# LeonhardFeiner/sparse_rcnn

Measured on AMD Instinct MI355X. Metric: active-voxels/sec fwd+bwd, ScanNet U-Net backbone, higher is better.
Workload: dtype f32

## Files before the change

### include/scn_mi355x.h

```cpp
#ifndef SCN_MI355X_H
#define SCN_MI355X_H

#include <stdint.h>

#ifdef __cplusplus
extern "C" {
#endif

#define SCN_OK 0
#define SCN_EINVAL 1
#define SCN_ESIZE 2
#define SCN_EHASH 3
#define SCN_EHIP 4

#define SCN_ABI_VERSION 5

#define SCN_F_RELU_IN 1
#define SCN_F_W_TRANSPOSED 2
#define SCN_F_OFF_REVERSE 4
#define SCN_F_RESIDUAL_LAST 8
#define SCN_F_SPLIT_SUM 16
#define SCN_F_TILE_ORDER_X 64
#define SCN_F_GEMM_V1 32

// ... 136 lines not shown
                         int flags, scn_stream_t stream);
int scn_wgrad_bias_rules_bf16(const uint16_t* X, int cin, const uint16_t* dY, int cout, const int32_t* in_rows,
                              const int32_t* out_rows, const int64_t* prefix_host, int n_off, float* dW, float* db,
                              uint32_t db_offsets, void* scratch, int flags, scn_stream_t stream);
int scn_wgrad_bias_rules(const float* X, int cin, const float* dY, int cout, const int32_t* in_rows,
                         const int32_t* out_rows, const int64_t* prefix_host, int n_off, float* dW, float* db,
                         uint32_t db_offsets, void* scratch, int flags, scn_stream_t stream);

int scn_wgrad_defer_begin(void);
int scn_wgrad_defer_flush(scn_stream_t stream);
int scn_wgrad_step_begin(void);
int scn_wgrad_step_hold(int on);
int scn_wgrad_step_flush(scn_stream_t stream);
int scn_wgrad_step_discard(void);
void scn_wgrad_group_counts(int64_t out[4], int reset);
int64_t scn_wgrad_scratch_bytes2(int cin, int cout, const int64_t* prefix_host, int n_off);
int scn_wgrad_bias_rules2(const float* X0, const float* dY0, const float* X1, const float* dY1, int cin, int cout,
                          const int32_t* in_rows, const int32_t* out_rows, const int64_t* prefix_host, int n_off,
                          float* dW, float* db, uint32_t db_offsets, void* scratch, int flags, scn_stream_t stream);

int64_t scn_wgrad_scratch_bytes_n(int cin, int cout, const int64_t* prefix_host, int n_off, int n_prob);
int scn_wgrad_bias_rules_n(const float* const* Xs, const float* const* dYs, int n_prob, int cin, int cout,
                          const int32_t* in_rows, const int32_t* out_rows, const int64_t* prefix_host, int n_off,
                          float* dW, float* db, uint32_t db_offsets, void* scratch, int flags, scn_stream_t stream);
int scn_wgrad_bias_rules_n_bf16(const uint16_t* const* Xs, const uint16_t* const* dYs, int n_prob, int cin, int cout,
                               const int32_t* in_rows, const int32_t* out_rows, const int64_t* prefix_host, int n_off,
                               float* dW, float* db, uint32_t db_offsets, void* scratch, int flags, scn_stream_t stream);
int scn_wgrad_bias_rules2_bf16(const uint16_t* X0, const uint16_t* dY0, const uint16_t* X1, const uint16_t* dY1, int cin,
                               int cout, const int32_t* in_rows, const int32_t* out_rows, const int64_t* prefix_host,
                               int n_off, float* dW, float* db, uint32_t db_offsets, void* scratch, int flags,
// ... 311 lines not shown
```

### sparse_rcnn_amd/_lib.py

```python
from __future__ import annotations

import ctypes as C
import os

import torch

_HERE = os.path.dirname(os.path.abspath(__file__))
LIB_PATH = os.environ.get("SCN_MI355X_LIB") or os.path.join(_HERE, "libscn_mi355x.so")

_lib = None

p = C.c_void_p
i32, i64, f32 = C.c_int, C.c_int64, C.c_float

_SIGS = {
    "scn_abi_version": (C.c_int, []),
    "scn_last_error_string": (C.c_char_p, []),
    "scn_debug_set": (C.c_int, [C.c_char_p, C.c_char_p]),
    "scn_debug_get": (C.c_int, [C.c_char_p, C.POINTER(C.c_int), C.POINTER(i64)]),
    "scn_hash_capacity": (i64, [i64]),
    "scn_coords_to_i32": (C.c_int, [p, i64, p, p, C.POINTER(i64), p]),
    "scn_dedup_scratch_bytes": (i64, [i64]),
    "scn_dedup_build": (C.c_int, [p, i64, i32, p, p, i64, p, p, p, p, p, C.POINTER(i64), p]),
    "scn_dedup_launch": (C.c_int, [p, i64, i32, p, p, i64, p, p, p, p, p, p, p]),
# ... 42 lines not shown
    "scn_wgrad_rules": (C.c_int, [p, i32, p, i32, p, p, C.POINTER(i64), i32, p, p, i32, p]),
    "scn_gemm_table_bf16": (C.c_int, [p, i64, i32, p, i32, i64, p, p, p, p, p, i32, i32, p]),
    "scn_gemm_rules_bf16": (C.c_int, [p, i32, p, p, C.POINTER(i64), i32, p, p, p, p, i32, i32, p]),
    "scn_gemm_rows2": (C.c_int, [p, i32, p, i32, i64, p, p, p, p, p, i32, p, i32, i32, i32, p]),
    "scn_wgrad_rules_bf16": (C.c_int, [p, i32, p, i32, p, p, C.POINTER(i64), i32, p, p, i32, p]),
    "scn_wgrad_bias_rules": (C.c_int, [p, i32, p, i32, p, p, C.POINTER(i64), i32, p, p, C.c_uint32, p, i32, p]),
    "scn_wgrad_bias_rules_bf16": (C.c_int, [p, i32, p, i32, p, p, C.POINTER(i64), i32, p, p, C.c_uint32, p, i32, p]),
    "scn_wgrad_scratch_bytes2": (i64, [i32, i32, C.POINTER(i64), i32]),
    "scn_wgrad_defer_begin": (C.c_int, []),
    "scn_wgrad_defer_flush": (C.c_int, [p]),
    "scn_wgrad_step_begin": (C.c_int, []),
    "scn_wgrad_step_hold": (C.c_int, [i32]),
    "scn_wgrad_step_flush": (C.c_int, [p]),
    "scn_wgrad_step_discard": (C.c_int, []),
    "scn_wgrad_group_counts": (None, [C.POINTER(i64), i32]),
    "scn_wgrad_bias_rules2": (C.c_int, [p, p, p, p, i32, i32, p, p, C.POINTER(i64), i32, p, p, C.c_uint32, p, i32, p]),
    "scn_wgrad_bias_rules2_bf16": (C.c_int, [p, p, p, p, i32, i32, p, p, C.POINTER(i64), i32, p, p, C.c_uint32, p, i32, p]),
    "scn_wgrad_scratch_bytes_n": (i64, [i32, i32, C.POINTER(i64), i32, i32]),
    "scn_wgrad_bias_rules_n": (C.c_int, [C.POINTER(p), C.POINTER(p), i32, i32, i32, p, p, C.POINTER(i64), i32, p, p, C.c_uint32, p, i32, p]),
    "scn_wgrad_bias_rules_n_bf16": (C.c_int, [C.POINTER(p), C.POINTER(p), i32, i32, i32, p, p, C.POINTER(i64), i32, p, p, C.c_uint32, p, i32, p]),
    "scn_colsum": (C.c_int, [p, i64, i32, p, p, p]),
    "scn_colsum_bf16": (C.c_int, [p, i64, i32, p, p, p]),
    "scn_relu_fwd": (C.c_int, [p, i64, p, p]),
    "scn_relu_bwd": (C.c_int, [p, p, i64, p, p]),
    "scn_add": (C.c_int, [p, p, i64, p, p]),
    "scn_bn_scratch_bytes": (i64, [i32]),
    "scn_bn_stats": (C.c_int, [p, i64, i32, p, p, p, p]),
    "scn_bn_sums": (C.c_int, [p, i64, i32, p, p, p]),
    "scn_bn_bwd_reduce": (C.c_int, [p, p, i64, i32, p, p, f32, p, p, f32, p, p, p, p, p]),
    "scn_bn_bwd_apply": (C.c_int, [p, p, i64, i32, p, p, f32, p, p, f32, p, i64, p, p]),
# ... 212 lines not shown
```

### sparse_rcnn_amd/csrc/scn_common.h

```cpp
#pragma once
#include <hip/hip_runtime.h>
#include <atomic>
#include <stdint.h>
#include <stdio.h>
#include <string.h>

#include "../../include/scn_mi355x.h"

namespace scn {

extern thread_local char g_err[512];

inline int fail(int code, const char* fmt, const char* a = "", long long b = 0, long long c = 0) {
    snprintf(g_err, sizeof(g_err), fmt, a, b, c);
    return code;
}

#define SCN_HIP(expr)                                                                               \
    do {                                                                                            \
        hipError_t e_ = (expr);                                                                     \
        if (e_ != hipSuccess) {                                                                     \
            snprintf(scn::g_err, sizeof(scn::g_err), "%s failed: %s (%s:%d)", #expr,                \
                     hipGetErrorString(e_), __FILE__, __LINE__);                                    \
            return SCN_EHIP;                                                                        \
// ... 10 lines not shown
        }                                                                                           \
    } while (0)

#define SCN_REQUIRE(cond)                                                                           \
    do {                                                                                            \
        if (!(cond)) {                                                                              \
            snprintf(scn::g_err, sizeof(scn::g_err), "%s: requirement failed: %s", __func__, #cond); \
            return SCN_EINVAL;                                                                      \
        }                                                                                           \
    } while (0)

enum Switch {
    SW_TS_SPLIT, SW_TS_SPLIT_MAX, SW_TS_NO_TAIL, SW_TS_W_HALF, SW_TS_W_BOTH, SW_TB_NB, SW_TB_KH, SW_TB_STREAM,
    SW_TB_NO_XORDER, SW_TS_STREAM, SW_TSS_NW, SW_EXEC_DEFER_SUMS, SW_PYRAMID_V1, SW_PYRAMID_ONE_STREAM, SW_WD_NO_T3,
    SW_WGRAD_BF16_MFMA, SW_WGRAD_SPLITS, SW_WD_NO_EVEC, SW_PYRAMID_NO_BRICKS, SW_CU_BUDGET, SW_EXP_A, SW_EXP_B, SW_TS_NO_CHAIN, SW_TS_PROG, SW_TB_NO_BINS,
    SW_EXEC_GROUP_WGRAD, SW_EXEC_GROUP_STEP, SW_COUNT
};
struct SwitchVal { bool set = false; long long i = 0; double f = 0.0; };
SwitchVal sw(Switch s);
inline int cu_budget() { const SwitchVal v = sw(SW_CU_BUDGET); return (v.set && v.i >= 32 && v.i <= 256) ? (int)v.i : 256; }

struct DeviceOnce {
    std::atomic<uint64_t> mask{0};
    static int cur() { int d = 0; return (hipGetDevice(&d) == hipSuccess && d >= 0 && d < 64) ? d : -1; }
    bool needed() const { const int d = cur(); return d < 0 || !(mask.load(std::memory_order_acquire) & (1ull << d)); }
    void done() { const int d = cur(); if (d >= 0) mask.fetch_or(1ull << d, std::memory_order_release); }
};

int wgrad_defer_group(bool on);

inline hipStream_t S(scn_stream_t s) { return reinterpret_cast<hipStream_t>(s); }
// ... 44 lines not shown
```

### sparse_rcnn_amd/csrc/scn_debug.hip

```cpp
#include <stdlib.h>

#include <mutex>

#include "scn_common.h"

namespace scn {
namespace {
struct Entry { const char* name; SwitchVal v; };
Entry g_sw[SW_COUNT] = {
    {"SCN_TS_SPLIT", {}},        {"SCN_TS_SPLIT_MAX", {}},  {"SCN_TS_NO_TAIL", {}},       {"SCN_TS_W_HALF", {}},
    {"SCN_TS_W_BOTH", {}},       {"SCN_TB_NB", {}},         {"SCN_TB_KH", {}},            {"SCN_TB_STREAM", {}},
    {"SCN_TB_NO_XORDER", {}},    {"SCN_TS_STREAM", {}},     {"SCN_TSS_NW", {}},           {"SCN_EXEC_DEFER_SUMS", {}},
    {"SCN_PYRAMID_V1", {}},      {"SCN_PYRAMID_ONE_STREAM", {}}, {"SCN_WD_NO_T3", {}},    {"SCN_WGRAD_BF16_MFMA", {}},
    {"SCN_WGRAD_SPLITS", {}},    {"SCN_WD_NO_EVEC", {}},    {"SCN_PYRAMID_NO_BRICKS", {}},            {"SCN_CU_BUDGET", {}},
    {"SCN_EXP_A", {}},           {"SCN_EXP_B", {}},         {"SCN_TS_NO_CHAIN", {}},
    {"SCN_TS_PROG", {}},         {"SCN_TB_NO_BINS", {}},    {"SCN_EXEC_GROUP_WGRAD", {}},
    {"SCN_EXEC_GROUP_STEP", {}},
};
std::once_flag g_once;
std::mutex g_mu;

void assign(SwitchVal& v, const char* s) {
    v.set = s != nullptr;
    v.i = s ? atoll(s) : 0;
    v.f = s ? atof(s) : 0.0;
}
void load_env() {
    for (int k = 0; k < SW_COUNT; ++k) assign(g_sw[k].v, getenv(g_sw[k].name));
}
}

SwitchVal sw(Switch s) {
// ... 30 lines not shown
```

### sparse_rcnn_amd/csrc/scn_wgrad.hip

```cpp
#include <stdlib.h>

#include <string.h>
#include <mutex>
#include <vector>

#include "scn_common.h"

#ifndef WD_DEEP_ALL
#define WD_DEEP_ALL 1
#endif

using scn::S;
using scn::cdiv;

typedef float f32x4 __attribute__((ext_vector_type(4)));
#define MFMA16(a, b, c) __builtin_amdgcn_mfma_f32_16x16x4f32((a), (b), (c), 0, 0, 0)

#ifndef WD_EXP
#define WD_EXP 0
#endif
#ifndef WD_TIMELINE
#define WD_TIMELINE 0
#endif
#if WD_TIMELINE
// ... 43 lines not shown
            f[2 * j] = __uint_as_float(r[j] << 16);
            f[2 * j + 1] = __uint_as_float(r[j] & 0xffff0000u);
        }
    } else {
        f = r;
    }
    return f;
}

__device__ __forceinline__ void wd_range(const DPlan& plan, int ov, int o, int prob, long long& p_lo, long long& p_hi) {
    const long long p_shift = prob * plan.p_rules;
    p_lo = plan.rule_start[ov] - p_shift;
    p_hi = plan.rule_start[ov + 1] - p_shift;
}

template <int TA, int TB, bool QUAD, bool EDGE, bool IDENT, bool HB = false>
__global__ __launch_bounds__(256) void k_wgrad_direct(const float* __restrict__ X_0, int cin, const float* __restrict__ dY_0,
                                                      int cout, const int* __restrict__ in_rows,
                                                      const int* __restrict__ out_rows, DPlan plan,
                                                      float* __restrict__ slabs, int relu_in,
                                                      float* __restrict__ db_slabs, unsigned db_mask, int cout_pad,
                                                      WdOps more) {
    const int unit = blockIdx.x, zb = blockIdx.z;
#include "scn_wgrad_unit.inc"
}

#define WG_MAX_JOBS 6
#define WG_MAXV 54
#define WG_MAXR 27
struct GJob {
    const void* X[2]; const void* dY[2];
    const int* in_rows; const int* out_rows;
    float* slabs; float* db_slabs;
    long long per;
    int cin, cout, relu_in, cout_pad, n_off, n_real, nbi, nbj, units, kind;
    unsigned db_mask;
    int unit_start[WG_MAXV + 1];
    long long prefix[WG_MAXR + 1];
};
struct GroupJobs { int n; int block_start[WG_MAX_JOBS + 1]; GJob job[WG_MAX_JOBS]; };

__device__ __forceinline__ int wd_offset_of(const GJob& j, int unit, int lane) {
    const bool lo = lane < j.n_off && unit >= j.unit_start[lane + 1];
    return __builtin_amdgcn_readfirstlane(__popcll(__ballot(lo)));
}
__device__ __forceinline__ void wd_range(const GJob& j, int ov, int o, int prob, long long& p_lo, long long& p_hi) {
    p_lo = j.prefix[o];
    p_hi = j.prefix[o + 1];
}

#define WD_KIND(TA_, TB_, Q_, E_, I_, H_) \
    ((TA_) | ((TB_) << 3) | ((Q_) ? 1 << 6 : 0) | ((E_) ? 1 << 7 : 0) | ((I_) ? 1 << 8 : 0) | ((H_) ? 1 << 9 : 0))

// ... 5 lines not shown
    return j;
}
#define WG_CONST(T_, p_) ((const __attribute__((address_space(4))) T_*)(p_))
__device__ __forceinline__ int wg_find(const GroupTable& t, int b) {
    int lo = 0, hi = t.n;
    while (hi - lo > 1) {
        const int mid = (lo + hi) >> 1;
        if (b >= WG_CONST(int, t.block_start)[mid]) lo = mid; else hi = mid;
    }
    return lo;
}
__device__ __forceinline__ const GJob& wg_job(const GroupJobs& g, int j) { return g.job[j]; }
__device__ __forceinline__ int wg_start(const GroupJobs& g, int j) { return g.block_start[j]; }
__device__ __forceinline__ const GJob& wg_job(const GroupTable& t, int j) { return *(const GJob*)(WG_CONST(GJob, t.job) + j); }
__device__ __forceinline__ int wg_start(const GroupTable& t, int j) { return WG_CONST(int, t.block_start)[j]; }

template <int VAR, typename SRC = GroupJobs>
__global__ __launch_bounds__(256) __attribute__((amdgpu_waves_per_eu(VAR, VAR))) void k_wgrad_group(SRC g) {
    const int j = wg_find(g, (int)blockIdx.x);
    const GJob& J = wg_job(g, j);
    const int local = (int)blockIdx.x - wg_start(g, j);
    const int zb = local / J.units, unit = local - zb * J.units;
    const float* __restrict__ X_0 = (const float*)J.X[0];
    const float* __restrict__ dY_0 = (const float*)J.dY[0];
    const int cin = J.cin, cout = J.cout, relu_in = J.relu_in, cout_pad = J.cout_pad;
    const int* __restrict__ in_rows = J.in_rows;
    const int* __restrict__ out_rows = J.out_rows;
    float* __restrict__ slabs = J.slabs;
    float* __restrict__ db_slabs = J.db_slabs;
    const unsigned db_mask = J.db_mask;
    const GJob& plan = J;
    const GJob& more = J;
#define WG_UNIT(TA_, TB_, Q_, I_) \
    constexpr int TA = TA_, TB = TB_;  \
    constexpr bool QUAD = Q_, EDGE = false, IDENT = I_, HB = false;
    if constexpr (VAR == 4) {
        switch (J.kind) {
        case WD_KIND(2, 2, false, false, false, false): {
            WG_UNIT(2, 2, false, false)
#include "scn_wgrad_unit.inc"
        } break;
        case WD_KIND(2, 2, false, false, true, false): {
            WG_UNIT(2, 2, false, true)
#include "scn_wgrad_unit.inc"
        } break;
        default: break;
        }
    } else {
        switch (J.kind) {
        case WD_KIND(2, 2, false, false, false, false): {
// ... 36 lines not shown
            WG_UNIT(4, 4, false, true)
#include "scn_wgrad_unit.inc"
        } break;
        case WD_KIND(4, 4, true, false, false, false): {
            WG_UNIT(4, 4, true, false)
#include "scn_wgrad_unit.inc"
        } break;
        case WD_KIND(4, 4, true, false, true, false): {
            WG_UNIT(4, 4, true, true)
#include "scn_wgrad_unit.inc"
        } break;
        default: break;
        }
    }
#undef WG_UNIT
}


typedef short s16x4 __attribute__((ext_vector_type(4)));
typedef short s16x8 __attribute__((ext_vector_type(8)));
typedef __bf16 bf16x8 __attribute__((ext_vector_type(8)));
#define MFMAB32(a, b, c) __builtin_amdgcn_mfma_f32_16x16x32_bf16((a), (b), (c), 0, 0, 0)

__device__ __forceinline__ int wtb_off(int row, int ch) { return 256 * row + 16 * (ch ^ (((row & 3) << 2) | ((row >> 2) & 3))); }

template <int TA, int TB, bool IDENT>
__global__ __launch_bounds__(256) void k_wgrad_tb(const unsigned short* __restrict__ X_0, int cin,
                                                  const unsigned short* __restrict__ dY_0, int cout,
                                                  const int* __restrict__ in_rows, const int* __restrict__ out_rows,
                                                  DPlan plan, float* __restrict__ slabs, int relu_in,
// ... 148 lines not shown
                slab[(16 * (wi * TA + a) + 4 * kq + j) * CBJ + 16 * (wj * TB + b) + i] = acc[a][b][j];
    if (do_db && kq == 0) {
#pragma unroll
        for (int b = 0; b < TB; ++b) {
            const int c = co0 + 16 * (wj * TB + b) + i;
            if (c < cout_pad) db_slabs[(long long)unit * cout_pad + c] = dbacc[b][0];
        }
    }
}

struct SumArgs {
    const float* slabs; float* dW; const float* db_slabs; float* db;
    int unit_start[129];
    int n_off, n_real, cbi, cbj, nbi, nbj, cin, cout, cout_pad, main_blocks, G;
    unsigned db_mask;
};

template <int V, typename A>
__device__ __forceinline__ void wgradd_sum_body(const A& a, int block) {
    typedef typename Frag<V>::type vec_t;
    const float* __restrict__ slabs = a.slabs;
    const int cin = a.cin, cout = a.cout, G = a.G;
    if (block >= a.main_blocks) {
        const int cidx = block - a.main_blocks;
        const int prob = cidx / cout, co = cidx - prob * cout;
        float s = 0.f;
        for (int o = 0; o < a.n_real; ++o) {
            if (!((a.db_mask >> o) & 1u)) continue;
            const int ov = prob * a.n_real + o;
            for (int u = a.unit_start[ov] + threadIdx.x; u < a.unit_start[ov + 1]; u += 256)
                s += a.db_slabs[(long long)u * a.cout_pad + co];
        }
#pragma unroll
        for (int d = 32; d >= 1; d >>= 1) s += __shfl_down(s, d);
        __shared__ float w[4];
        if ((threadIdx.x & 63) == 0) w[threadIdx.x >> 6] = s;
        __syncthreads();
        if (threadIdx.x == 0) a.db[cidx] = (w[0] + w[1]) + (w[2] + w[3]);
        return;
    }
    __shared__ __attribute__((aligned(16))) float part[256 * V];
    const int per_block = 256 / G;
    const int el = threadIdx.x % per_block, g = threadIdx.x / per_block;
    const long long total = (long long)a.n_off * cin * (cout / V);
    const int cbi = a.cbi, cbj = a.cbj, nblk = a.nbi * a.nbj;
    const long long eg = (long long)block * per_block + el;
    vec_t sum;
#pragma unroll
    for (int v = 0; v < V; ++v) sum[v] = 0.f;
    long long e = 0;
    if (eg < total) {
        e = eg * V;
        const int co = (int)(e % cout);
// ... 137 lines not shown
    pl.p_rules = P;
    return rc;
}

namespace {
struct WdLaunch {
    DPlan pl;
    int ta, tb;
    bool quad, edge, ident, hb;
    const float* X; const float* dY;
    int cin, cout, relu_in, cout_pad, n_prob;
    const int32_t* in_rows; const int32_t* out_rows;
    float* slabs; float* db_slabs;
    unsigned db_mask;
    WdOps more;
    int kind() const { return WD_KIND(ta, tb, quad, edge, ident, hb); }
    int units() const { return pl.unit_start[pl.n_off]; }
    int64_t workgroups() const { return (int64_t)units() * pl.nbi * pl.nbj; }
    double wg_work() const { return (double)pl.per * pl.cbi * pl.cbj; }
    size_t lds() const { return (quad ? 4 * 64 : 4 * ta * tb * 4 * 64 + 4 * 64) * sizeof(float); }
};

std::atomic<int64_t> g_counts[4];

int launch_direct(const WdLaunch& r, scn_stream_t stream) {
    g_counts[2].fetch_add(1, std::memory_order_relaxed);
    const dim3 grid((unsigned)r.units(), 1, (unsigned)(r.pl.nbi * r.pl.nbj));
    const bool ident = r.ident, edge = r.edge, hb = r.hb;
#define LAUNCH_WD(TA_, TB_, Q_, E_, I_, H_)                                                                      \
    do {                                                                                                         \
        const size_t lds_ = ((Q_) ? 4 * 64 : 4 * (TA_) * (TB_) * 4 * 64 + 4 * 64) * sizeof(float);               \
        static scn::DeviceOnce attr_set;                                                                            \
        if (attr_set.needed()) {                                                                                         \
// ... 35 lines not shown
    std::vector<SumArgs> jobs; std::vector<int> blocks;
    std::vector<WdLaunch> units;
};
thread_local DeferState g_defer;

struct StepState {
    bool open = false, hold = false;
    std::vector<SumArgs> jobs; std::vector<int> blocks;
    std::vector<WdLaunch> units;
    void clear() { jobs.clear(); blocks.clear(); units.clear(); }
};
thread_local StepState g_step;

struct TableRing {
    static constexpr int N = 4;
    struct Slot { char* host = nullptr; char* dev = nullptr; size_t cap = 0; hipEvent_t ev = nullptr; bool busy = false; };
    std::mutex mu;
    Slot slot[N];
    int next = 0;
    int release(Slot& s) {
        if (s.busy) SCN_HIP(hipEventSynchronize(s.ev));
        s.busy = false;
        if (s.host) SCN_HIP(hipHostFree(s.host));
        s.host = nullptr;
        if (s.dev) SCN_HIP(hipFree(s.dev));
        s.dev = nullptr;
        s.cap = 0;
        return SCN_OK;
    }
    int take(size_t bytes, Slot** out) {
        Slot& s = slot[next];
        next = (next + 1) % N;
        if (!s.ev) SCN_HIP(hipEventCreateWithFlags(&s.ev, hipEventDisableTiming));
        if (s.busy) SCN_HIP(hipEventSynchronize(s.ev));
        s.busy = false;
        if (s.cap < bytes) {
            const int rc = release(s);
            if (rc != SCN_OK) return rc;
            const size_t cap = (bytes + 65535) & ~(size_t)65535;
            SCN_HIP(hipHostMalloc((void**)&s.host, cap, hipHostMallocDefault));
            SCN_HIP(hipMalloc((void**)&s.dev, cap));
            s.cap = cap;
// ... 5 lines not shown
constexpr int RING_DEVICES = 64;
TableRing g_rings[RING_DEVICES];

void fill_gjob(const WdLaunch& r, GJob& J) {
    for (int p = 0; p < 2; ++p) {
        J.X[p] = p == 0 ? (const void*)r.X : (r.n_prob > 1 ? r.more.X[p] : nullptr);
        J.dY[p] = p == 0 ? (const void*)r.dY : (r.n_prob > 1 ? r.more.dY[p] : nullptr);
    }
    J.in_rows = r.in_rows; J.out_rows = r.out_rows; J.slabs = r.slabs; J.db_slabs = r.db_slabs;
    J.per = r.pl.per;
    J.cin = r.cin; J.cout = r.cout; J.relu_in = r.relu_in; J.cout_pad = r.cout_pad;
    J.n_off = r.pl.n_off; J.n_real = r.pl.n_real; J.nbi = r.pl.nbi; J.nbj = r.pl.nbj;
    J.units = r.units(); J.kind = r.kind(); J.db_mask = r.db_mask;
    for (int v = 0; v <= r.pl.n_off; ++v) J.unit_start[v] = r.pl.unit_start[v];
    for (int o = 0; o <= r.pl.n_real; ++o) J.prefix[o] = r.pl.rule_start[o];
}

void sort_members(const std::vector<WdLaunch>& R, std::vector<int>& members) {
    std::stable_sort(members.begin(), members.end(), [&](int a, int b) {
        if (R[a].wg_work() != R[b].wg_work()) return R[a].wg_work() > R[b].wg_work();
        return R[a].workgroups() > R[b].workgroups();
    });
}

template <typename SRC>
int launch_group(int var, const SRC& g, unsigned blocks, size_t lds, scn_stream_t stream) {
    if (var == 4) {
        g_counts[0].fetch_add(1, std::memory_order_relaxed);
        hipLaunchKernelGGL((k_wgrad_group<4, SRC>), dim3(blocks), dim3(256), lds, S(stream), g);
    } else {
        static scn::DeviceOnce attr_set;
// ... 55 lines not shown
        if (v == 4) m4.push_back((int)k);
        else if (v == 2) m2.push_back((int)k);
    }
    if (m2.size() < 2) m2.clear();
    if (m4.size() < 2) m4.clear();
    std::vector<char> grouped(R.size(), 0);
    for (int k : m2) grouped[k] = 1;
    for (int k : m4) grouped[k] = 1;
    for (size_t k = 0; k < R.size(); ++k)
        if (!grouped[k]) {
            const int rc = launch_direct(R[k], stream);
            if (rc != SCN_OK) return rc;
        }
    sort_members(R, m2);
    sort_members(R, m4);
    const size_t n2 = m2.size(), n4 = m4.size(), ns = g_step.jobs.size();
    if (n2 + n4 + ns == 0) return SCN_OK;
    auto up = [](size_t b) { return (b + 63) & ~(size_t)63; };
    const size_t o2 = 0, o4 = up(o2 + n2 * sizeof(GJob)), os = up(o4 + n4 * sizeof(GJob));
    const size_t b2 = up(os + ns * sizeof(SumArgs)), b4 = up(b2 + (n2 + 1) * sizeof(int));
    const size_t bs = up(b4 + (n4 + 1) * sizeof(int)), bytes = up(bs + (ns + 1) * sizeof(int));
    int dev_id = 0;
    SCN_HIP(hipGetDevice(&dev_id));
    SCN_REQUIRE(dev_id >= 0 && dev_id < RING_DEVICES);
    TableRing& ring = g_rings[dev_id];
    std::lock_guard<std::mutex> ring_lock(ring.mu);
    TableRing::Slot* slot = nullptr;
    int rc = ring.take(bytes, &slot);
    if (rc != SCN_OK) return rc;
    char* h = slot->host;
    memset(h, 0, bytes);
    size_t lds2 = 0, lds4 = 0;
    int* s2 = (int*)(h + b2);
    for (size_t q = 0; q < n2; ++q) {
        const WdLaunch& r = R[m2[q]];
        fill_gjob(r, ((GJob*)(h + o2))[q]);
        s2[q + 1] = s2[q] + (int)r.workgroups();
        if (r.lds() > lds2) lds2 = r.lds();
    }
    int* s4 = (int*)(h + b4);
    for (size_t q = 0; q < n4; ++q) {
        const WdLaunch& r = R[m4[q]];
        fill_gjob(r, ((GJob*)(h + o4))[q]);
        s4[q + 1] = s4[q] + (int)r.workgroups();
        if (r.lds() > lds4) lds4 = r.lds();
    }
    int* ss = (int*)(h + bs);
    for (size_t q = 0; q < ns; ++q) {
        memcpy(h + os + q * sizeof(SumArgs), &g_step.jobs[q], sizeof(SumArgs));
        ss[q + 1] = ss[q] + g_step.blocks[q];
    }
    SCN_HIP(hipMemcpyAsync(slot->dev, h, bytes, hipMemcpyHostToDevice, S(stream)));
    const char* d = slot->dev;
    if (n2) {
        GroupTable t{(const GJob*)(d + o2), (const int*)(d + b2), (int)n2};
        rc = launch_group(2, t, (unsigned)s2[n2], lds2, stream);
    }
    if (rc == SCN_OK && n4) {
        GroupTable t{(const GJob*)(d + o4), (const int*)(d + b4), (int)n4};
        rc = launch_group(4, t, (unsigned)s4[n4], lds4, stream);
    }
    if (rc == SCN_OK && ns) {
        g_counts[3].fetch_add(1, std::memory_order_relaxed);
        hipLaunchKernelGGL(k_wgradd_sum_many_tab, dim3((unsigned)ss[ns]), dim3(256), 0, S(stream),
                           (const SumArgs*)(d + os), (const int*)(d + bs), (int)ns);
// ... 44 lines not shown
        if (db) SCN_HIP(hipMemsetAsync(db, 0, sizeof(float) * (size_t)n_prob * cout, S(stream)));
        return SCN_OK;
    }
    const Shape sh = pick_shape(cin, cout, hb);
    const bool edge = (cin % (16 * sh.ta) != 0) || (cout % (16 * sh.tb) != 0) ||
                      ((all_ptrs & (sh.ta == 3 ? 3 : 15)) != 0);
    const bool ident = in_rows == nullptr;
    const int cout_pad = pl.nbj * pl.cbj;
    float* db_slabs = db ? (float*)scratch + (int64_t)pl.unit_start[n_off] * pl.nbi * pl.nbj * pl.cbi * pl.cbj : nullptr;
    dim3 grid((unsigned)pl.unit_start[n_off], 1, (unsigned)(pl.nbi * pl.nbj));
    const bool evec = edge && !hb && cin % sh.ta == 0 && cout % sh.tb == 0 && (all_ptrs & 15) == 0 &&
                      (cin * 4) % 16 == 0 && (cout * 4) % 16 == 0 && !scn::sw(scn::SW_WD_NO_EVEC).set;
    const int relu_in = ((flags & SCN_F_RELU_IN) ? 1 : 0) | (evec ? 2 : 0);
    const int V = (cout % 4 == 0 && (((uintptr_t)dW | (uintptr_t)scratch) & 15) == 0) ? 4 : 1;
    const bool deferred = g_defer.on && V == 4;
    if (mfma16) {
        const int ta = tb_tiles(cin), tb = tb_tiles(cout);
#define LAUNCH_WT(TA_, TB_, I_)                                                                                  \
    hipLaunchKernelGGL((k_wgrad_tb<TA_, TB_, I_>), grid, dim3(256), 4 * 32 * 256, S(stream), (const unsigned short*)X, cin, \
                       (const unsigned short*)dY, cout, in_rows, out_rows, pl, (float*)scratch, relu_in, db_slabs, db_mask, \
                       cout_pad, more)
#define PICK_WT(TA_, TB_) do { if (ident) LAUNCH_WT(TA_, TB_, true); else LAUNCH_WT(TA_, TB_, false); } while (0)
        if (ta == 1 && tb == 1) PICK_WT(1, 1);
        else if (ta == 1 && tb == 2) PICK_WT(1, 2);
        else if (ta == 1 && tb == 4) PICK_WT(1, 4);
        else if (ta == 2 && tb == 1) PICK_WT(2, 1);
        else if (ta == 2 && tb == 2) PICK_WT(2, 2);
        else if (ta == 2 && tb == 4) PICK_WT(2, 4);
        else if (ta == 4 && tb == 1) PICK_WT(4, 1);
        else if (ta == 4 && tb == 2) PICK_WT(4, 2);
        else PICK_WT(4, 4);
#undef PICK_WT
#undef LAUNCH_WT
        SCN_LAUNCH_CHECK();
        g_counts[2].fetch_add(1, std::memory_order_relaxed);
    } else {
        WdLaunch r;
        r.pl = pl;
        r.ta = sh.ta; r.tb = sh.tb; r.quad = sh.quad; r.edge = edge; r.ident = ident; r.hb = hb;
        if (sh.ta == 3) r.edge = false;
        r.X = X; r.dY = dY; r.cin = cin; r.cout = cout; r.relu_in = relu_in; r.cout_pad = cout_pad; r.n_prob = n_prob;
        r.in_rows = in_rows; r.out_rows = out_rows; r.slabs = (float*)scratch; r.db_slabs = db_slabs; r.db_mask = db_mask;
        r.more = more;
        if (deferred && g_defer.group) g_defer.units.push_back(r);
        else {
            const int rc = launch_direct(r, stream);
            if (rc != SCN_OK) return rc;
        }
    }
    const int64_t groups = (int64_t)n_off * cin * (cout / V);
    int G = 1;
    while (G < 16 && groups * G < 128 * 1024) G *= 2;
    SumArgs sa;
    sa.slabs = (const float*)scratch; sa.dW = dW; sa.db_slabs = db_slabs; sa.db = db;
    memcpy(sa.unit_start, pl.unit_start, sizeof(sa.unit_start));
    sa.n_off = pl.n_off; sa.n_real = pl.n_real; sa.cbi = pl.cbi; sa.cbj = pl.cbj; sa.nbi = pl.nbi; sa.nbj = pl.nbj;
    sa.cin = cin; sa.cout = cout; sa.cout_pad = cout_pad; sa.main_blocks = (int)cdiv(groups, 256 / G); sa.G = G;
    sa.db_mask = db_mask;
    const int blocks = sa.main_blocks + (db ? n_prob * cout : 0);
    if (deferred) {
        g_defer.jobs.push_back(sa);
        g_defer.blocks.push_back(blocks);
        return SCN_OK;
    }
    if (V == 4) hipLaunchKernelGGL(k_wgradd_sum<4>, dim3(blocks), dim3(256), 0, S(stream), sa);
    else hipLaunchKernelGGL(k_wgradd_sum<1>, dim3(blocks), dim3(256), 0, S(stream), sa);
    SCN_LAUNCH_CHECK();
    g_counts[3].fetch_add(1, std::memory_order_relaxed);
    return SCN_OK;
}

extern "C" int scn_wgrad_defer_begin(void) {
    g_defer.on = true;
    g_defer.group = false;
    g_defer.jobs.clear();
    g_defer.blocks.clear();
    g_defer.units.clear();
    return SCN_OK;
}

extern "C" int scn_wgrad_defer_flush(scn_stream_t stream) {
    SCN_REQUIRE(g_defer.on);
    g_defer.on = false;
    g_defer.group = false;
    if (g_step.open && g_step.hold) {
        g_step.units.insert(g_step.units.end(), g_defer.units.begin(), g_defer.units.end());
        g_step.jobs.insert(g_step.jobs.end(), g_defer.jobs.begin(), g_defer.jobs.end());
        g_step.blocks.insert(g_step.blocks.end(), g_defer.blocks.begin(), g_defer.blocks.end());
        g_defer.units.clear();
        g_defer.jobs.clear();
        g_defer.blocks.clear();
        return SCN_OK;
    }
    int rc = flush_units(stream);
    g_defer.units.clear();
    const size_t n = g_defer.jobs.size();
    for (size_t base = 0; rc == SCN_OK && base < n; base += WD_SUM_MANY) {
        SumJobs jobs;
        jobs.n = (int)(n - base < WD_SUM_MANY ? n - base : WD_SUM_MANY);
        jobs.block_start[0] = 0;
// ... 34 lines not shown
}

extern "C" int scn_wgrad_step_discard(void) {
    g_step.open = g_step.hold = false;
    g_step.clear();
    return SCN_OK;
}

extern "C" void scn_wgrad_group_counts(int64_t out[4], int reset) {
    for (int k = 0; k < 4; ++k) {
        if (out) out[k] = g_counts[k].load(std::memory_order_relaxed);
        if (reset) g_counts[k].store(0, std::memory_order_relaxed);
    }
}

extern "C" int scn_wgrad_rules(const float* X, int cin, const float* dY, int cout, const int32_t* in_rows,
                               const int32_t* out_rows, const int64_t* prefix_host, int n_off, float* dW, void* scratch,
                               int flags, scn_stream_t stream) {
    return wgrad_impl(X, cin, dY, cout, in_rows, out_rows, prefix_host, n_off, dW, nullptr, 0u, scratch, flags, stream);
}

extern "C" int scn_wgrad_rules_bf16(const uint16_t* X, int cin, const uint16_t* dY, int cout, const int32_t* in_rows,
                                    const int32_t* out_rows, const int64_t* prefix_host, int n_off, float* dW,
                                    void* scratch, int flags, scn_stream_t stream) {
    return wgrad_impl((const float*)X, cin, (const float*)dY, cout, in_rows, out_rows, prefix_host, n_off, dW, nullptr,
                      0u, scratch, flags, stream, true);
}

extern "C" int scn_wgrad_bias_rules(const float* X, int cin, const float* dY, int cout, const int32_t* in_rows,
                                    const int32_t* out_rows, const int64_t* prefix_host, int n_off, float* dW, float* db,
// ... 72 lines not shown
```

### sparse_rcnn_amd/csrc/scn_wgrad_unit.inc

```
{
    typedef typename Frag<TA>::type fa_t;
    typedef typename Frag<TB>::type fb_t;
    constexpr bool PACKED = HB && !EDGE;
    typedef typename RawFrag<TA, PACKED>::type ra_t;
    typedef typename RawFrag<TB, PACKED>::type rb_t;
    constexpr int ES = HB ? 2 : 4;
    constexpr int WI = 16 * TA, WJ = 16 * TB;
    constexpr int CBI = QUAD ? 2 * WI : WI, CBJ = QUAD ? 2 * WJ : WJ;
    constexpr int NACC = TA * TB;
    extern __shared__ __attribute__((aligned(16))) float red[];

    const int tid = threadIdx.x, lane = tid & 63;
    const int wave = __builtin_amdgcn_readfirstlane(tid >> 6);
#if WD_TIMELINE
    const long long wd_t0 = wall_clock64();
#endif
    const int i = lane & 15, kq = lane >> 4;
    const int ov = wd_offset_of(plan, unit, lane);
    const int prob = ov / plan.n_real;
    const int o = ov - prob * plan.n_real;
    const float* X = prob ? (const float*)more.X[prob] : X_0;
    const float* dY = prob ? (const float*)more.dY[prob] : dY_0;
    const int s_unit = unit - plan.unit_start[ov];
    const int bi = zb / plan.nbj, bj = zb % plan.nbj;
// ... 190 lines not shown
            for (int b = 0; b < TB; ++b)
#pragma unroll
                for (int j = 0; j < 4; ++j) mine[((a * TB + b) * 4 + j) * 64 + lane] = acc[a][b][j];
        __syncthreads();
#pragma unroll
        for (int jj = 0; jj < TA; ++jj) {
            const int p_own = wave * TA + jj;
            const int a_own = p_own >> 2, jx = p_own & 3;
            fb_t v;
#pragma unroll
            for (int b = 0; b < TB; ++b) {
                const float* src = red + ((a_own * TB + b) * 4 + jx) * 64 + lane;
                v[b] = ((src[0] + src[NACC * 4 * 64]) + src[2 * NACC * 4 * 64]) + src[3 * NACC * 4 * 64];
            }
            const int r = TA * (4 * kq + jx) + a_own;
            *(fb_t*)(slab + r * CBJ + TB * i) = v;
        }
    } else {
#pragma unroll
        for (int a = 0; a < TA; ++a)
#pragma unroll
            for (int j = 0; j < 4; ++j) {
                const int r = wi * WI + TA * (4 * kq + j) + a;
                fb_t v;
#pragma unroll
                for (int b = 0; b < TB; ++b) v[b] = acc[a][b][j];
                *(fb_t*)(slab + r * CBJ + wj * WJ + TB * i) = v;
            }
    }

    if (db_slabs != nullptr && ((db_mask >> o) & 1u) && bi == 0) {
#pragma unroll
        for (int t = 0; t < TB; ++t) {
            float v = dbacc[t];
            v += __shfl_xor(v, 16);
            v += __shfl_xor(v, 32);
            dbacc[t] = v;
        }
        if (!QUAD) {
            if (kq == 0) {
#pragma unroll
                for (int t = 0; t < TB; ++t) dbr[wave * 64 + TB * i + t] = dbacc[t];
// ... 25 lines not shown
```

Before: 28.57 million.

## Fold wgrad slab reduction into grouped launch via last-arriver atomic counters

In the grouped wgrad kernel, each workgroup writes its partial slab with write-through buffer stores, then bumps a per-(offset,tile) atomic counter. The last arriving workgroup sums all unit slabs and writes dW directly. The separate sum kernel then only zeroes dW for offsets with no rules. The aim is to drop most of the separate reduction pass and its launch or serialization cost, at the price of atomics, a vmcnt wait, and a serialized tail reduction done by a single workgroup per tile.

Result: slower. 25.74 million (-9.9%).

```diff
diff --git a/include/scn_mi355x.h b/include/scn_mi355x.h
--- a/include/scn_mi355x.h
+++ b/include/scn_mi355x.h
@@ -174,6 +174,7 @@
 int scn_wgrad_step_flush(scn_stream_t stream);
 int scn_wgrad_step_discard(void);
 void scn_wgrad_group_counts(int64_t out[4], int reset);
+int scn_wgrad_sum_in_launch_counts(int64_t out[4], int reset);
 int64_t scn_wgrad_scratch_bytes2(int cin, int cout, const int64_t* prefix_host, int n_off);
 int scn_wgrad_bias_rules2(const float* X0, const float* dY0, const float* X1, const float* dY1, int cin, int cout,
                           const int32_t* in_rows, const int32_t* out_rows, const int64_t* prefix_host, int n_off,
diff --git a/sparse_rcnn_amd/_lib.py b/sparse_rcnn_amd/_lib.py
--- a/sparse_rcnn_amd/_lib.py
+++ b/sparse_rcnn_amd/_lib.py
@@ -80,6 +80,7 @@
     "scn_wgrad_step_flush": (C.c_int, [p]),
     "scn_wgrad_step_discard": (C.c_int, []),
     "scn_wgrad_group_counts": (None, [C.POINTER(i64), i32]),
+    "scn_wgrad_sum_in_launch_counts": (C.c_int, [C.POINTER(i64), i32]),
     "scn_wgrad_bias_rules2": (C.c_int, [p, p, p, p, i32, i32, p, p, C.POINTER(i64), i32, p, p, C.c_uint32, p, i32, p]),
     "scn_wgrad_bias_rules2_bf16": (C.c_int, [p, p, p, p, i32, i32, p, p, C.POINTER(i64), i32, p, p, C.c_uint32, p, i32, p]),
     "scn_wgrad_scratch_bytes_n": (i64, [i32, i32, C.POINTER(i64), i32, i32]),
diff --git a/sparse_rcnn_amd/csrc/scn_common.h b/sparse_rcnn_amd/csrc/scn_common.h
--- a/sparse_rcnn_amd/csrc/scn_common.h
+++ b/sparse_rcnn_amd/csrc/scn_common.h
@@ -48,7 +48,7 @@
     SW_TS_SPLIT, SW_TS_SPLIT_MAX, SW_TS_NO_TAIL, SW_TS_W_HALF, SW_TS_W_BOTH, SW_TB_NB, SW_TB_KH, SW_TB_STREAM,
     SW_TB_NO_XORDER, SW_TS_STREAM, SW_TSS_NW, SW_EXEC_DEFER_SUMS, SW_PYRAMID_V1, SW_PYRAMID_ONE_STREAM, SW_WD_NO_T3,
     SW_WGRAD_BF16_MFMA, SW_WGRAD_SPLITS, SW_WD_NO_EVEC, SW_PYRAMID_NO_BRICKS, SW_CU_BUDGET, SW_EXP_A, SW_EXP_B, SW_TS_NO_CHAIN, SW_TS_PROG, SW_TB_NO_BINS,
-    SW_EXEC_GROUP_WGRAD, SW_EXEC_GROUP_STEP, SW_COUNT
+    SW_EXEC_GROUP_WGRAD, SW_EXEC_GROUP_STEP, SW_WGRAD_SUM_IN_LAUNCH, SW_COUNT
 };
 struct SwitchVal { bool set = false; long long i = 0; double f = 0.0; };
 SwitchVal sw(Switch s);
diff --git a/sparse_rcnn_amd/csrc/scn_debug.hip b/sparse_rcnn_amd/csrc/scn_debug.hip
--- a/sparse_rcnn_amd/csrc/scn_debug.hip
+++ b/sparse_rcnn_amd/csrc/scn_debug.hip
@@ -15,7 +15,7 @@
     {"SCN_WGRAD_SPLITS", {}},    {"SCN_WD_NO_EVEC", {}},    {"SCN_PYRAMID_NO_BRICKS", {}},            {"SCN_CU_BUDGET", {}},
     {"SCN_EXP_A", {}},           {"SCN_EXP_B", {}},         {"SCN_TS_NO_CHAIN", {}},
     {"SCN_TS_PROG", {}},         {"SCN_TB_NO_BINS", {}},    {"SCN_EXEC_GROUP_WGRAD", {}},
-    {"SCN_EXEC_GROUP_STEP", {}},
+    {"SCN_EXEC_GROUP_STEP", {}},   {"SCN_WGRAD_SUM_IN_LAUNCH", {}},
 };
 std::once_flag g_once;
 std::mutex g_mu;
diff --git a/sparse_rcnn_amd/csrc/scn_wgrad.hip b/sparse_rcnn_amd/csrc/scn_wgrad.hip
--- a/sparse_rcnn_amd/csrc/scn_wgrad.hip
+++ b/sparse_rcnn_amd/csrc/scn_wgrad.hip
@@ -81,6 +81,20 @@
     p_hi = plan.rule_start[ov + 1] - p_shift;
 }
 
+typedef unsigned u32x2 __attribute__((ext_vector_type(2)));
+typedef unsigned u32x4 __attribute__((ext_vector_type(4)));
+template <bool WT, int TB>
+__device__ __forceinline__ void wd_store(float* slab, int block_floats, int at, const typename Frag<TB>::type& v) {
+    if constexpr (WT) {
+        static_assert(TB == 2 || TB == 4, "write-through slab stores are 8 or 16 bytes per lane");
+        const __amdgpu_buffer_rsrc_t rs = __builtin_amdgcn_make_buffer_rsrc((void*)slab, 0, block_floats * 4, 0x00020000);
+        if constexpr (TB == 4) __builtin_amdgcn_raw_buffer_store_b128(__builtin_bit_cast(u32x4, v), rs, at * 4, 0, 16);
+        else __builtin_amdgcn_raw_buffer_store_b64(__builtin_bit_cast(u32x2, v), rs, at * 4, 0, 16);
+    } else {
+        *(typename Frag<TB>::type*)(slab + at) = v;
+    }
+}
+
 template <int TA, int TB, bool QUAD, bool EDGE, bool IDENT, bool HB = false>
 __global__ __launch_bounds__(256) void k_wgrad_direct(const float* __restrict__ X_0, int cin, const float* __restrict__ dY_0,
                                                       int cout, const int* __restrict__ in_rows,
@@ -89,6 +103,7 @@
                                                       float* __restrict__ db_slabs, unsigned db_mask, int cout_pad,
                                                       WdOps more) {
     const int unit = blockIdx.x, zb = blockIdx.z;
+    constexpr bool WT = false;
 #include "scn_wgrad_unit.inc"
 }
 
@@ -104,6 +119,7 @@
     unsigned db_mask;
     int unit_start[WG_MAXV + 1];
     long long prefix[WG_MAXR + 1];
+    int* ctr; float* dW; int G;
 };
 struct GroupJobs { int n; int block_start[WG_MAX_JOBS + 1]; GJob job[WG_MAX_JOBS]; };
 
@@ -139,6 +155,60 @@
 __device__ __forceinline__ int wg_start(const GroupJobs& g, int j) { return g.block_start[j]; }
 __device__ __forceinline__ const GJob& wg_job(const GroupTable& t, int j) { return *(const GJob*)(WG_CONST(GJob, t.job) + j); }
 __device__ __forceinline__ int wg_start(const GroupTable& t, int j) { return WG_CONST(int, t.block_start)[j]; }
+
+template <typename SRC> struct WgTable { static constexpr bool value = false; };
+template <> struct WgTable<GroupTable> { static constexpr bool value = true; };
+
+__device__ __forceinline__ void wg_sum_in_launch(const GJob& J, int unit, int zb) {
+    extern __shared__ __attribute__((aligned(16))) float wg_red[];
+    const int tid = threadIdx.x, lane = tid & 63;
+    asm volatile("s_waitcnt vmcnt(0)" ::: "memory");
+    __syncthreads();
+    const int ov = wd_offset_of(J, unit, lane);
+    const int u0 = J.unit_start[ov], nu = J.unit_start[ov + 1] - u0;
+    const int nblk = J.nbi * J.nbj;
+    if (nu > 1) {
+        if (tid == 0) {
+            typedef __attribute__((address_space(1))) int gint;
+            gint* ctr = (gint*)(J.ctr + ov * nblk + zb);
+            const int t = __hip_atomic_fetch_add(ctr, 1, __ATOMIC_RELAXED, __HIP_MEMORY_SCOPE_AGENT);
+            if (t == nu - 1) __hip_atomic_store(ctr, 0, __ATOMIC_RELAXED, __HIP_MEMORY_SCOPE_AGENT);
+            ((int*)wg_red)[0] = t;
+        }
+        __syncthreads();
+        if (__builtin_amdgcn_readfirstlane(((const int*)wg_red)[0]) != nu - 1) return;
+    }
+    __builtin_amdgcn_fence(__ATOMIC_ACQUIRE, "wavefront");
+    const int quad = (J.kind >> 6) & 1;
+    const int cbi = (16 * (J.kind & 7)) << quad, cbj = (16 * ((J.kind >> 3) & 7)) << quad;
+    const int cb = cbi * cbj;
+    const int bi = zb / J.nbj, bj = zb - bi * J.nbj;
+    const int G = J.G;
+    const int ustride = nblk * cb * 4;
+    const float* first = J.slabs + ((long long)u0 * nblk + zb) * cb;
+    const __amdgpu_buffer_rsrc_t rs = __builtin_amdgcn_make_buffer_rsrc((void*)first, 0, (nu - 1) * ustride + cb * 4, 0x00020000);
+    float* out = J.dW + ((long long)ov * J.cin + bi * cbi) * J.cout + bj * cbj;
+    for (int e = 4 * tid; e < cb; e += 1024) {
+        f32x4 sum = {0.f, 0.f, 0.f, 0.f};
+        for (int g = 0; g < G; ++g) {
+            f32x4 chain = {0.f, 0.f, 0.f, 0.f};
+            for (int s = g; s < nu; s += 4 * G) {
+                f32x4 p[4];
+#pragma unroll
+                for (int u = 0; u < 4; ++u) {
+                    const int su = s + u * G < nu ? s + u * G : s;
+                    p[u] = __builtin_bit_cast(f32x4, __builtin_amdgcn_raw_buffer_load_b128(rs, su * ustride + e * 4, 0, 16));
+                }
+#pragma unroll
+                for (int u = 0; u < 4; ++u)
+                    if (s + u * G < nu) chain += p[u];
+            }
+            if (g == 0) sum = chain; else sum += chain;
+        }
+        const int r = e / cbj, c = e - r * cbj;
+        if (bi * cbi + r < J.cin && bj * cbj + c < J.cout) *(f32x4*)(out + (long long)r * J.cout + c) = sum;
+    }
+}
 
 template <int VAR, typename SRC = GroupJobs>
 __global__ __launch_bounds__(256) __attribute__((amdgpu_waves_per_eu(VAR, VAR))) void k_wgrad_group(SRC g) {
@@ -158,7 +228,7 @@
     const GJob& more = J;
 #define WG_UNIT(TA_, TB_, Q_, I_) \
     constexpr int TA = TA_, TB = TB_;  \
-    constexpr bool QUAD = Q_, EDGE = false, IDENT = I_, HB = false;
+    constexpr bool QUAD = Q_, EDGE = false, IDENT = I_, HB = false, WT = WgTable<SRC>::value && TB_ != 3;
     if constexpr (VAR == 4) {
         switch (J.kind) {
         case WD_KIND(2, 2, false, false, false, false): {
@@ -225,6 +295,9 @@
         }
     }
 #undef WG_UNIT
+    if constexpr (WgTable<SRC>::value) {
+        if (J.ctr != nullptr) wg_sum_in_launch(J, unit, zb);
+    }
 }
 
 
@@ -403,6 +476,8 @@
     int unit_start[129];
     int n_off, n_real, cbi, cbj, nbi, nbj, cin, cout, cout_pad, main_blocks, G;
     unsigned db_mask;
+    int in_launch;
+    unsigned long long empty;
 };
 
 template <int V, typename A>
@@ -426,6 +501,18 @@
         if ((threadIdx.x & 63) == 0) w[threadIdx.x >> 6] = s;
         __syncthreads();
         if (threadIdx.x == 0) a.db[cidx] = (w[0] + w[1]) + (w[2] + w[3]);
+        return;
+    }
+    if (a.in_launch) {
+        const int gpo = cin * (cout / V), bpo = (gpo + 255) / 256;
+        const int k = block / bpo, eg = (block - k * bpo) * 256 + (int)threadIdx.x;
+        unsigned long long m = a.empty;
+        for (int q = 0; q < k; ++q) m &= m - 1;
+        const int o = __ffsll(m) - 1;
+        vec_t zero;
+#pragma unroll
+        for (int v = 0; v < V; ++v) zero[v] = 0.f;
+        if (eg < gpo) *(vec_t*)(a.dW + ((long long)o * gpo + eg) * V) = zero;
         return;
     }
     __shared__ __attribute__((aligned(16))) float part[256 * V];
@@ -593,9 +680,12 @@
     float* slabs; float* db_slabs;
     unsigned db_mask;
     WdOps more;
+    float* dW; int G;
+    int sum_job;
     int kind() const { return WD_KIND(ta, tb, quad, edge, ident, hb); }
     int units() const { return pl.unit_start[pl.n_off]; }
     int64_t workgroups() const { return (int64_t)units() * pl.nbi * pl.nbj; }
+    int64_t slab_bytes() const { return workgroups() * pl.cbi * pl.cbj * (int64_t)sizeof(float); }
     double wg_work() const { return (double)pl.per * pl.cbi * pl.cbj; }
     size_t lds() const { return (quad ? 4 * 64 : 4 * ta * tb * 4 * 64 + 4 * 64) * sizeof(float); }
 };
@@ -661,7 +751,10 @@
 
 struct TableRing {
     static constexpr int N = 4;
-    struct Slot { char* host = nullptr; char* dev = nullptr; size_t cap = 0; hipEvent_t ev = nullptr; bool busy = false; };
+    struct Slot {
+        char* host = nullptr; char* dev = nullptr; size_t cap = 0; hipEvent_t ev = nullptr; bool busy = false;
+        int* ctr = nullptr; size_t n_ctr = 0;
+    };
     std::mutex mu;
     Slot slot[N];
     int next = 0;
@@ -673,6 +766,20 @@
         if (s.dev) SCN_HIP(hipFree(s.dev));
         s.dev = nullptr;
         s.cap = 0;
+        if (s.ctr) SCN_HIP(hipFree(s.ctr));
+        s.ctr = nullptr;
+        s.n_ctr = 0;
+        return SCN_OK;
+    }
+    int counters(Slot& s, size_t n, hipStream_t stream) {
+        if (s.n_ctr >= n) return SCN_OK;
+        if (s.ctr) SCN_HIP(hipFree(s.ctr));
+        s.ctr = nullptr;
+        s.n_ctr = 0;
+        const size_t cap = (n + 4095) & ~(size_t)4095;
+        SCN_HIP(hipMalloc((void**)&s.ctr, cap * sizeof(int)));
+        SCN_HIP(hipMemsetAsync(s.ctr, 0, cap * sizeof(int), stream));
+        s.n_ctr = cap;
         return SCN_OK;
     }
     int take(size_t bytes, Slot** out) {
@@ -708,7 +815,16 @@
     J.units = r.units(); J.kind = r.kind(); J.db_mask = r.db_mask;
     for (int v = 0; v <= r.pl.n_off; ++v) J.unit_start[v] = r.pl.unit_start[v];
     for (int o = 0; o <= r.pl.n_real; ++o) J.prefix[o] = r.pl.rule_start[o];
-}
+    J.ctr = nullptr; J.dW = r.dW; J.G = r.G;
+}
+
+bool sums_in_launch(const WdLaunch& r) {
+    const scn::SwitchVal v = scn::sw(scn::SW_WGRAD_SUM_IN_LAUNCH);
+    if (v.set && v.i == 0) return false;
+    return r.ta != 3 && r.sum_job >= 0 && r.dW != nullptr && r.slab_bytes() < ((int64_t)1 << 31);
+}
+
+std::atomic<int64_t> g_sil[3];
 
 void sort_members(const std::vector<WdLaunch>& R, std::vector<int>& members) {
     std::stable_sort(members.begin(), members.end(), [&](int a, int b) {
@@ -794,7 +910,35 @@
         }
     sort_members(R, m2);
     sort_members(R, m4);
-    const size_t n2 = m2.size(), n4 = m4.size(), ns = g_step.jobs.size();
+    std::vector<SumArgs> sums(g_step.jobs);
+    std::vector<int> sum_blocks(g_step.blocks);
+    std::vector<long long> ctr_at(R.size(), -1);
+    size_t n_ctr = 0;
+    for (const std::vector<int>* m : {&m2, &m4})
+        for (int k : *m) {
+            const WdLaunch& r = R[k];
+            if (!sums_in_launch(r) || r.sum_job >= (int)sums.size()) continue;
+            SumArgs& sa = sums[r.sum_job];
+            SCN_REQUIRE(sa.slabs == r.slabs && sa.dW == r.dW && sa.G == r.G && sa.n_off == r.pl.n_off);
+            ctr_at[k] = (long long)n_ctr;
+            n_ctr += (size_t)r.pl.n_off * r.pl.nbi * r.pl.nbj;
+            int n_empty = 0, most = 0;
+            for (int v = 0; v < r.pl.n_off; ++v) {
+                const int nu = r.pl.unit_start[v + 1] - r.pl.unit_start[v];
+                if (nu == 0) { sa.empty |= 1ull << v; ++n_empty; }
+                if (nu > most) most = nu;
+            }
+            const int main_was = sa.main_blocks;
+            sa.in_launch = 1;
+            sa.main_blocks = n_empty * (int)cdiv((int64_t)r.cin * (r.cout / 4), 256);
+            sum_blocks[r.sum_job] += sa.main_blocks - main_was;
+            g_sil[0].fetch_add(1, std::memory_order_relaxed);
+            if (r.G > 1 && most > r.G) g_sil[1].fetch_add(1, std::memory_order_relaxed);
+            g_sil[2].fetch_add(n_empty, std::memory_order_relaxed);
+        }
+    for (size_t q = sums.size(); q-- > 0;)
+        if (sum_blocks[q] == 0) { sums.erase(sums.begin() + q); sum_blocks.erase(sum_blocks.begin() + q); }
+    const size_t n2 = m2.size(), n4 = m4.size(), ns = sums.size();
     if (n2 + n4 + ns == 0) return SCN_OK;
     auto up = [](size_t b) { return (b + 63) & ~(size_t)63; };
     const size_t o2 = 0, o4 = up(o2 + n2 * sizeof(GJob)), os = up(o4 + n4 * sizeof(GJob));
@@ -808,6 +952,10 @@
     TableRing::Slot* slot = nullptr;
     int rc = ring.take(bytes, &slot);
     if (rc != SCN_OK) return rc;
+    if (n_ctr) {
+        rc = ring.counters(*slot, n_ctr, S(stream));
+        if (rc != SCN_OK) return rc;
+    }
     char* h = slot->host;
     memset(h, 0, bytes);
     size_t lds2 = 0, lds4 = 0;
@@ -815,6 +963,7 @@
     for (size_t q = 0; q < n2; ++q) {
         const WdLaunch& r = R[m2[q]];
         fill_gjob(r, ((GJob*)(h + o2))[q]);
+        if (ctr_at[m2[q]] >= 0) ((GJob*)(h + o2))[q].ctr = slot->ctr + ctr_at[m2[q]];
         s2[q + 1] = s2[q] + (int)r.workgroups();
         if (r.lds() > lds2) lds2 = r.lds();
     }
@@ -822,13 +971,14 @@
     for (size_t q = 0; q < n4; ++q) {
         const WdLaunch& r = R[m4[q]];
         fill_gjob(r, ((GJob*)(h + o4))[q]);
+        if (ctr_at[m4[q]] >= 0) ((GJob*)(h + o4))[q].ctr = slot->ctr + ctr_at[m4[q]];
         s4[q + 1] = s4[q] + (int)r.workgroups();
         if (r.lds() > lds4) lds4 = r.lds();
     }
     int* ss = (int*)(h + bs);
     for (size_t q = 0; q < ns; ++q) {
-        memcpy(h + os + q * sizeof(SumArgs), &g_step.jobs[q], sizeof(SumArgs));
-        ss[q + 1] = ss[q] + g_step.blocks[q];
+        memcpy(h + os + q * sizeof(SumArgs), &sums[q], sizeof(SumArgs));
+        ss[q + 1] = ss[q] + sum_blocks[q];
     }
     SCN_HIP(hipMemcpyAsync(slot->dev, h, bytes, hipMemcpyHostToDevice, S(stream)));
     const char* d = slot->dev;
@@ -903,6 +1053,9 @@
     const int relu_in = ((flags & SCN_F_RELU_IN) ? 1 : 0) | (evec ? 2 : 0);
     const int V = (cout % 4 == 0 && (((uintptr_t)dW | (uintptr_t)scratch) & 15) == 0) ? 4 : 1;
     const bool deferred = g_defer.on && V == 4;
+    const int64_t groups = (int64_t)n_off * cin * (cout / V);
+    int G = 1;
+    while (G < 16 && groups * G < 128 * 1024) G *= 2;
     if (mfma16) {
         const int ta = tb_tiles(cin), tb = tb_tiles(cout);
 #define LAUNCH_WT(TA_, TB_, I_)                                                                                  \
@@ -931,21 +1084,20 @@
         r.X = X; r.dY = dY; r.cin = cin; r.cout = cout; r.relu_in = relu_in; r.cout_pad = cout_pad; r.n_prob = n_prob;
         r.in_rows = in_rows; r.out_rows = out_rows; r.slabs = (float*)scratch; r.db_slabs = db_slabs; r.db_mask = db_mask;
         r.more = more;
+        r.dW = dW; r.G = G; r.sum_job = deferred ? (int)g_defer.jobs.size() : -1;
         if (deferred && g_defer.group) g_defer.units.push_back(r);
         else {
             const int rc = launch_direct(r, stream);
             if (rc != SCN_OK) return rc;
         }
     }
-    const int64_t groups = (int64_t)n_off * cin * (cout / V);
-    int G = 1;
-    while (G < 16 && groups * G < 128 * 1024) G *= 2;
     SumArgs sa;
     sa.slabs = (const float*)scratch; sa.dW = dW; sa.db_slabs = db_slabs; sa.db = db;
     memcpy(sa.unit_start, pl.unit_start, sizeof(sa.unit_start));
     sa.n_off = pl.n_off; sa.n_real = pl.n_real; sa.cbi = pl.cbi; sa.cbj = pl.cbj; sa.nbi = pl.nbi; sa.nbj = pl.nbj;
     sa.cin = cin; sa.cout = cout; sa.cout_pad = cout_pad; sa.main_blocks = (int)cdiv(groups, 256 / G); sa.G = G;
     sa.db_mask = db_mask;
+    sa.in_launch = 0; sa.empty = 0;
     const int blocks = sa.main_blocks + (db ? n_prob * cout : 0);
     if (deferred) {
         g_defer.jobs.push_back(sa);
@@ -973,6 +1125,8 @@
     g_defer.on = false;
     g_defer.group = false;
     if (g_step.open && g_step.hold) {
+        for (WdLaunch& r : g_defer.units)
+            if (r.sum_job >= 0) r.sum_job += (int)g_step.jobs.size();
         g_step.units.insert(g_step.units.end(), g_defer.units.begin(), g_defer.units.end());
         g_step.jobs.insert(g_step.jobs.end(), g_defer.jobs.begin(), g_defer.jobs.end());
         g_step.blocks.insert(g_step.blocks.end(), g_defer.blocks.begin(), g_defer.blocks.end());
@@ -1037,6 +1191,30 @@
     }
 }
 
+extern "C" int scn_wgrad_sum_in_launch_counts(int64_t out[4], int reset) {
+    for (int k = 0; k < 3; ++k) {
+        if (out) out[k] = g_sil[k].load(std::memory_order_relaxed);
+        if (reset) g_sil[k].store(0, std::memory_order_relaxed);
+    }
+    if (!out) return SCN_OK;
+    int dev_id = 0;
+    SCN_HIP(hipGetDevice(&dev_id));
+    SCN_REQUIRE(dev_id >= 0 && dev_id < RING_DEVICES);
+    TableRing& ring = g_rings[dev_id];
+    std::lock_guard<std::mutex> ring_lock(ring.mu);
+    SCN_HIP(hipDeviceSynchronize());
+    int64_t nonzero = 0;
+    std::vector<int> host;
+    for (TableRing::Slot& s : ring.slot) {
+        if (!s.ctr) continue;
+        host.resize(s.n_ctr);
+        SCN_HIP(hipMemcpy(host.data(), s.ctr, s.n_ctr * sizeof(int), hipMemcpyDeviceToHost));
+        for (int c : host) nonzero += c != 0;
+    }
+    out[3] = nonzero;
+    return SCN_OK;
+}
+
 extern "C" int scn_wgrad_rules(const float* X, int cin, const float* dY, int cout, const int32_t* in_rows,
                                const int32_t* out_rows, const int64_t* prefix_host, int n_off, float* dW, void* scratch,
                                int flags, scn_stream_t stream) {
diff --git a/sparse_rcnn_amd/csrc/scn_wgrad_unit.inc b/sparse_rcnn_amd/csrc/scn_wgrad_unit.inc
--- a/sparse_rcnn_amd/csrc/scn_wgrad_unit.inc
+++ b/sparse_rcnn_amd/csrc/scn_wgrad_unit.inc
@@ -228,7 +228,7 @@
                 v[b] = ((src[0] + src[NACC * 4 * 64]) + src[2 * NACC * 4 * 64]) + src[3 * NACC * 4 * 64];
             }
             const int r = TA * (4 * kq + jx) + a_own;
-            *(fb_t*)(slab + r * CBJ + TB * i) = v;
+            wd_store<WT, TB>(slab, CBI * CBJ, r * CBJ + TB * i, v);
         }
     } else {
 #pragma unroll
@@ -239,7 +239,7 @@
                 fb_t v;
 #pragma unroll
                 for (int b = 0; b < TB; ++b) v[b] = acc[a][b][j];
-                *(fb_t*)(slab + r * CBJ + wj * WJ + TB * i) = v;
+                wd_store<WT, TB>(slab, CBI * CBJ, r * CBJ + wj * WJ + TB * i, v);
             }
     }
 
```
